# bogus2000/anytime-3D-reconstruction

Measured on AMD Instinct MI355X. Metric: 32^3 voxel reconstructions/sec at batch=256; IoU delta vs reference, higher is better.
Workload: dtype bf16

## Files before the change

anytime-3d-reconstruction_amd/csrc/skip_direct.hip:

```cpp
#include "common.h"

namespace {

typedef __attribute__((ext_vector_type(4))) unsigned sd_u4;

constexpr int SD_ATILE = 256 * 128;
constexpr int SD_WST = 32768;
constexpr int SD_A0 = 4096;
constexpr int SD_W0 = SD_A0 + 2 * SD_ATILE;
constexpr int SD_ZERO = SD_W0 + 2 * SD_WST;
constexpr int SD_LDS = SD_ZERO + 4096;
constexpr int SD_XCH = 0;
constexpr int SD_OST = 65536;
constexpr int SD_OPITCH = 144;
constexpr int SD_TPITCH = 272;
constexpr int SD_TWAVE = 16 * SD_TPITCH;

struct SdArgs {
    const void *x;
    const void *w;
    const float *scale;
    const float *shift;
    void *y;
    int batch, cin, cout, act;
    unsigned x_bytes, w_bytes;
    int groups;
};

__global__ void sd_pack_conv_kernel(const float *__restrict__ w, __bf16 *__restrict__ out, int cin, int cout) {
    const int NC = cin / 64;
    const long total = (long)64 * cin * cout;
    for (long i = (long)blockIdx.x * blockDim.x + threadIdx.x; i < total; i += (long)gridDim.x * blockDim.x) {
        const int k = (int)(i & 63);
        long r = i >> 6;
        const int n = (int)(r % cout); r /= cout;
        const int c = (int)(r % NC);
        const int t = (int)(r / NC);
        out[i] = static_cast<__bf16>(w[((size_t)t * cin + c * 64 + k) * cout + n]);
    }
}

__device__ __forceinline__ void sd_pack_conv_tiled_body(const float *__restrict__ w, __bf16 *__restrict__ out, int cin, int cout, int kb, int nb) {
    __shared__ float tile[64][65];
    const int tid = threadIdx.x;
    const int n0 = nb * 64;
    const int c4 = tid & 15, r = tid >> 4;
#pragma unroll
    for (int j = 0; j < 4; ++j) {
        const int kl = r + 16 * j;
// ... 43 lines not shown
        const int n = (int)(r % cout); r /= cout;
        const int c = (int)(r % NC); r /= NC;
        const int a = (int)(r & 7), p = (int)(r >> 3);
        const int td = 1 - ((p >> 2) & 1) + 2 * ((a >> 2) & 1);
        const int th = 1 - ((p >> 1) & 1) + 2 * ((a >> 1) & 1);
        const int tw = 1 - (p & 1) + 2 * (a & 1);
        const int t = (td * 4 + th) * 4 + tw;
        const float *src = w + ((size_t)t * cout + n) * cin + c * 64 + k;
        const f32x4 v0 = *reinterpret_cast<const f32x4 *>(src), v1 = *reinterpret_cast<const f32x4 *>(src + 4);
        bf16x8 o;
#pragma unroll
        for (int u = 0; u < 4; ++u) { o[u] = static_cast<__bf16>(v0[u]); o[4 + u] = static_cast<__bf16>(v1[u]); }
        *reinterpret_cast<bf16x8 *>(out + i8 * 8) = o;
    }
}

__global__ void sd_pack_convT_kernel(const float *__restrict__ w, __bf16 *__restrict__ out, int cin, int cout) {
    sd_pack_convT_body(w, out, cin, cout, blockIdx.x, gridDim.x);
}

__global__ void sd_pack_convT_multi_kernel(const SdPackJobs t) {
    int j = 0;
    while (j + 1 < t.njobs && (int)blockIdx.x >= t.first[j + 1]) ++j;
    sd_pack_convT_body(t.w[j], t.out[j], t.cin[j], t.cout[j], (int)blockIdx.x - t.first[j], t.first[j + 1] - t.first[j]);
}

#define SD_RD(DST, ADDR, OFF) asm volatile("ds_read_b128 %0, %1 offset:%2" : "=v"(DST) : "v"(ADDR), "n"(OFF) : "memory")
#define SD_WAIT8(N, F, G)                                                                                                   \
    asm volatile("s_waitcnt lgkmcnt(%8)"                                                                                    \
                 : "+v"(F[0]), "+v"(F[1]), "+v"(F[2]), "+v"(F[3]), "+v"(G[0]), "+v"(G[1]), "+v"(G[2]), "+v"(G[3])          \
                 : "n"(N)                                                                                                   \
                 : "memory")

template <int MODE>
__global__ __launch_bounds__(512, 1) void sd_kernel(const SdArgs a) {
    extern __shared__ __attribute__((aligned(16))) char smem[];
    const int tid = threadIdx.x, lane = tid & 63;
    const int wave = __builtin_amdgcn_readfirstlane(tid >> 6);
    const int mq = wave & 3, hv = wave >> 2;
    const int NC = a.cin >> 6;

    const int nwg = gridDim.x;
    const int wi = (nwg & 7) ? (int)blockIdx.x : (int)(blockIdx.x & 7) * (nwg >> 3) + (int)(blockIdx.x >> 3);
    const int sg = wi / a.groups, g = wi - sg * a.groups;
    const int b0 = sg * 4;
    const int ng = MODE == 0 ? g : (g >> 2);
    const int pd = (g >> 1) & 1, ph = g & 1;

    const u32x4 rsx = vv_make_rsrc(a.x, a.x_bytes), rsw = vv_make_rsrc(a.w, a.w_bytes);
    const unsigned lds0 = (unsigned)(unsigned long long)(lptr_t)smem;

    for (int i = tid; i < 256; i += 512) reinterpret_cast<uint4 *>(smem + SD_ZERO)[i] = make_uint4(0, 0, 0, 0);
    __syncthreads();

    unsigned a_lane[4], w_lane[4];
#pragma unroll
    for (int k = 0; k < 4; ++k) {
        const int it = wave * 4 + k;
        const int R = it * 8 + (lane >> 3);
        const int s = R >> 6, jd = (R >> 4) & 3, jh = (R >> 2) & 3, jw = R & 3;
        const int slot = (lane & 7) ^ (((s & 1) << 2) | (jw & 2));
        if (MODE == 0) a_lane[k] = (unsigned)(((((b0 + s) * 8 + 2 * jd) * 8 + 2 * jh) * 8 + 2 * jw) * (a.cin * 2) + slot * 16);
        else a_lane[k] = (unsigned)((((b0 + s) * 64) + (R & 63)) * (a.cin * 2) + slot * 16);
        const int blk = MODE == 0 ? (it & 7) : (it & 15);
        const int nrow = blk * 8 + (lane >> 3);
        w_lane[k] = (unsigned)(nrow * 128 + (((lane & 7) ^ ((nrow >> 1) & 7)) << 4));
    }
    auto issue_a = [&](int T, int tq, int tc) {
        unsigned soff;
        if (MODE == 0) {
            const int q = tq, c = tc;
            soff = (unsigned)(((1 - ((q >> 2) & 1)) * 64 + (1 - ((q >> 1) & 1)) * 8 + (1 - (q & 1))) * (a.cin * 2) + c * 128);
        } else {
            soff = (unsigned)(T * 128);
        }
        soff = __builtin_amdgcn_readfirstlane(soff);
        const unsigned dst = lds0 + SD_A0 + (T & 1) * SD_ATILE + wave * 4096;
#pragma unroll
        for (int k = 0; k < 4; ++k) vv_dma16(rsx, a_lane[k], soff, dst + k * 1024);
    };
    auto issue_w = [&](int u, int tq, int tc) {
        unsigned soff;
        if (MODE == 0) {
            const int ad = u & 1;
            const int q = tq, c = tc;
            const int j = wave >> 1;
            const int td = 2 * ad + ((q >> 2) & 1), th = 2 * (j >> 1) + ((q >> 1) & 1), tw = 2 * (j & 1) + (q & 1);
            const int t = (td * 4 + th) * 4 + tw;
            soff = (unsigned)(((t * NC + c) * a.cout + ng * 64) * 128);
        } else {
            const int c = u >> 3, ta = u & 7;
            const int p = pd * 4 + ph * 2 + hv;
            soff = (unsigned)((((p * 8 + ta) * NC + c) * a.cout + ng * 128) * 128);
        }
        soff = __builtin_amdgcn_readfirstlane(soff);
        const unsigned dst = lds0 + SD_W0 + (u & 1) * SD_WST + wave * 4096;
#pragma unroll
        for (int k = 0; k < 4; ++k) vv_dma16(rsw, w_lane[k], soff, dst + k * 1024);
    };

    const int r = lane & 15, kq = lane >> 4, ls = r >> 2, lw = r & 3;
    auto arow = [&](int jw, int ks) -> unsigned {
        const int f = ((ls & 1) << 2) | (jw & 2);
        return (unsigned)((ls * 64 + jw) * 128 + ((((ks << 2) | kq) ^ f) << 4));
    };
    unsigned wb[2];
#pragma unroll
    for (int ks = 0; ks < 2; ++ks) wb[ks] = lds0 + SD_W0 + (unsigned)(r * 128 + ((((ks << 2) | kq) ^ ((r >> 1) & 7)) << 4));
    const unsigned wbc = hv ? wb[1] : wb[0];
    const unsigned wbt0 = wb[0] + (unsigned)(hv * 16384), wbt1 = wb[1] + (unsigned)(hv * 16384);

    int td_[4], th_[4];
#pragma unroll
    for (int i = 0; i < 4; ++i) { td_[i] = i; th_[i] = (i + mq) & 3; }

    constexpr int NT = MODE == 0 ? 4 : 8;
    f32x4 acc[4][NT];
#pragma unroll
    for (int i = 0; i < 4; ++i)
#pragma unroll
        for (int j = 0; j < NT; ++j) acc[i][j] = f32x4{0.f, 0.f, 0.f, 0.f};

    auto mma4 = [&](const sd_u4 *xf, const sd_u4 *wf, int nt0, int vmask, auto i_c) {
        constexpr int i = decltype(i_c)::value;
        if (vmask & (1 << i)) {
#pragma unroll
            for (int j = 0; j < 4; ++j)
                acc[i][nt0 + j] = __builtin_amdgcn_mfma_f32_16x16x32_bf16(*reinterpret_cast<const bf16x8 *>(&wf[j]),
                                                                           *reinterpret_cast<const bf16x8 *>(&xf[i]), acc[i][nt0 + j], 0, 0, 0);
        }
    };
#define SD_MMA_RD(XF, WF, NT0, VM, R1, R2)                                                                                  \
    do {                                                                                                                    \
        mma4(XF, WF, NT0, VM, std::integral_constant<int, 0>{});                                                            \
        R1;                                                                                                                 \
        mma4(XF, WF, NT0, VM, std::integral_constant<int, 1>{});                                                            \
        R2;                                                                                                                 \
        mma4(XF, WF, NT0, VM, std::integral_constant<int, 2>{});                                                            \
        mma4(XF, WF, NT0, VM, std::integral_constant<int, 3>{});                                                            \
    } while (0)
    auto tile_mask = [&](const int *cell, int off) -> int {
        int m = 0;
#pragma unroll
        for (int i = 0; i < 4; ++i) m |= ((unsigned)(cell[i] + off) < 4u) ? (1 << i) : 0;
        return __builtin_amdgcn_readfirstlane(m);
    };

    const int ntiles = MODE == 0 ? 8 * NC : NC;
    const int nunits = ntiles * (MODE == 0 ? 2 : 8);

    const int q1_ = NC > 1 ? 0 : 1, c1_ = NC > 1 ? 1 : 0;
    issue_a(0, 0, 0);
    issue_w(0, 0, 0);
    if (ntiles > 1) issue_a(1, q1_, c1_); else issue_a(0, 0, 0);
    issue_w(1, 0, 0);
    vv_wait_vm<8>();
    __builtin_amdgcn_s_barrier();

    auto zrow = [&](int jw, int ks) -> unsigned { return lds0 + SD_ZERO + (arow(jw & 3, ks) & 255u); };

    sd_u4 xP[4], xQ[4], wP[4], wQ[4];
    if constexpr (MODE == 0) {
        const unsigned lm1 = arow((lw - 1) & 3, hv), l00 = arow(lw, hv), lp1 = arow((lw + 1) & 3, hv);
        const unsigned zm1 = zrow(lw - 1, hv), zp1 = zrow(lw + 1, hv);
        const bool okm1 = lw >= 1, okp1 = lw <= 2;
        unsigned xb0[4], xb1[4];
        int dm0, dm1, hm0, hm1;
        auto setup = [&](int T, int q) {
            const int qd = (q >> 2) & 1, qh = (q >> 1) & 1, qw = q & 1;
            const unsigned abuf = lds0 + SD_A0 + (T & 1) * SD_ATILE;
#pragma unroll
            for (int i = 0; i < 4; ++i) {
                const unsigned sc_ = abuf + (unsigned)((td_[i] - 1 + qd) * 2048 + (th_[i] - 1 + qh) * 512);
                xb0[i] = qw ? l00 + sc_ : (okm1 ? lm1 + sc_ : zm1);
                xb1[i] = qw ? (okp1 ? lp1 + sc_ : zp1) : l00 + sc_;
            }
            dm0 = tile_mask(td_, qd - 1); dm1 = tile_mask(td_, qd); hm0 = tile_mask(th_, qh - 1); hm1 = tile_mask(th_, qh);
        };
#define SD_CONV_RD(AD, J, XF, WF)                                                                                           \
    do {                                                                                                                    \
        constexpr int XO = (AD) * 2048 + ((J) >> 1) * 512, WO = (AD) * SD_WST + (J) * 8192;                                 \
        if ((J) & 1) { SD_RD(XF[0], xb1[0], XO); SD_RD(XF[1], xb1[1], XO); SD_RD(XF[2], xb1[2], XO); SD_RD(XF[3], xb1[3], XO); } \
        else { SD_RD(XF[0], xb0[0], XO); SD_RD(XF[1], xb0[1], XO); SD_RD(XF[2], xb0[2], XO); SD_RD(XF[3], xb0[3], XO); }     \
        SD_RD(WF[0], wbc, WO); SD_RD(WF[1], wbc, WO + 2048); SD_RD(WF[2], wbc, WO + 4096); SD_RD(WF[3], wbc, WO + 6144);    \
    } while (0)
#define SD_CONV_RDX(AD, J, XF)                                                                                              \
    do {                                                                                                                    \
        constexpr int XO = (AD) * 2048 + ((J) >> 1) * 512;                                                                  \
        if ((J) & 1) { SD_RD(XF[0], xb1[0], XO); SD_RD(XF[1], xb1[1], XO); SD_RD(XF[2], xb1[2], XO); SD_RD(XF[3], xb1[3], XO); } \
        else { SD_RD(XF[0], xb0[0], XO); SD_RD(XF[1], xb0[1], XO); SD_RD(XF[2], xb0[2], XO); SD_RD(XF[3], xb0[3], XO); }     \
    } while (0)
#define SD_CONV_RDW(AD, J, WF)                                                                                              \
    do {                                                                                                                    \
        constexpr int WO = (AD) * SD_WST + (J) * 8192;                                                                      \
        SD_RD(WF[0], wbc, WO); SD_RD(WF[1], wbc, WO + 2048); SD_RD(WF[2], wbc, WO + 4096); SD_RD(WF[3], wbc, WO + 6144);    \
    } while (0)
        setup(0, 0);
        SD_CONV_RD(0, 0, xP, wP);
        int qa = 0, ca = 0;
        int qb = q1_, cb = c1_;
        int qc = cb + 1 < NC ? qb : qb + 1, cc = cb + 1 < NC ? cb + 1 : 0;
#pragma unroll 1
        for (int T = 0; T < ntiles; ++T) {
            {
                const int u = 2 * T;
                SD_WAIT8(0, xP, wP);
                SD_MMA_RD(xP, wP, 0, dm0 & hm0, SD_CONV_RDX(0, 1, xQ), SD_CONV_RDW(0, 1, wQ));
                SD_WAIT8(0, xQ, wQ);
                SD_MMA_RD(xQ, wQ, 0, dm0 & hm0, SD_CONV_RDX(0, 2, xP), SD_CONV_RDW(0, 2, wP));
                SD_WAIT8(0, xP, wP);
                SD_MMA_RD(xP, wP, 0, dm0 & hm1, SD_CONV_RDX(0, 3, xQ), SD_CONV_RDW(0, 3, wQ));
                SD_WAIT8(0, xQ, wQ);
                vv_wait_vm<0>();
                __builtin_amdgcn_s_barrier();
                SD_MMA_RD(xQ, wQ, 0, dm0 & hm1, if (u + 2 < nunits) issue_w(u + 2, qb, cb); SD_CONV_RDX(1, 0, xP), SD_CONV_RDW(1, 0, wP));
            }
            {
                const int u = 2 * T + 1;
                SD_WAIT8(0, xP, wP);
                SD_MMA_RD(xP, wP, 0, dm1 & hm0, SD_CONV_RDX(1, 1, xQ), SD_CONV_RDW(1, 1, wQ));
                SD_WAIT8(0, xQ, wQ);
                SD_MMA_RD(xQ, wQ, 0, dm1 & hm0, SD_CONV_RDX(1, 2, xP), SD_CONV_RDW(1, 2, wP));
                SD_WAIT8(0, xP, wP);
                SD_MMA_RD(xP, wP, 0, dm1 & hm1, SD_CONV_RDX(1, 3, xQ), SD_CONV_RDW(1, 3, wQ));
                SD_WAIT8(0, xQ, wQ);
                vv_wait_vm<0>();
                __builtin_amdgcn_s_barrier();
                const int lastmask = dm1 & hm1;
                mma4(xQ, wQ, 0, lastmask, std::integral_constant<int, 0>{});
                if (u + 2 < nunits) issue_w(u + 2, qb, cb);
                if (T + 2 < ntiles) issue_a(T + 2, qc, cc);
                mma4(xQ, wQ, 0, lastmask, std::integral_constant<int, 1>{});
                if (T + 1 < ntiles) {
                    setup(T + 1, qb);
                    SD_CONV_RD(0, 0, xP, wP);
                }
                mma4(xQ, wQ, 0, lastmask, std::integral_constant<int, 2>{});
                mma4(xQ, wQ, 0, lastmask, std::integral_constant<int, 3>{});
            }
            qa = qb; ca = cb; qb = qc; cb = cc;
            qc = cb + 1 < NC ? qb : qb + 1; cc = cb + 1 < NC ? cb + 1 : 0;
            (void)qa; (void)ca;
        }
        asm volatile("s_waitcnt lgkmcnt(0)" ::: "memory");
        __builtin_amdgcn_sched_barrier(0);
#undef SD_CONV_RD
#undef SD_CONV_RDX
#undef SD_CONV_RDW
    } else {
        const int jw0 = lw + hv, jw1 = lw + hv - 1;
        const unsigned l0[2] = {arow(jw0 & 3, 0), arow(jw0 & 3, 1)}, l1[2] = {arow(jw1 & 3, 0), arow(jw1 & 3, 1)};
        const unsigned z0[2] = {zrow(jw0, 0), zrow(jw0, 1)}, z1[2] = {zrow(jw1, 0), zrow(jw1, 1)};
        const bool ok0 = (unsigned)jw0 < 4u, ok1 = (unsigned)jw1 < 4u;
        int dmA[2] = {tile_mask(td_, pd), tile_mask(td_, pd - 1)};
        const int hmA[2] = {tile_mask(th_, ph), tile_mask(th_, ph - 1)};
        unsigned xb[2][2][4];
        auto setup = [&](int T) {
            const unsigned abuf = lds0 + SD_A0 + (T & 1) * SD_ATILE;
#pragma unroll
            for (int i = 0; i < 4; ++i) {
                const unsigned sc_ = abuf + (unsigned)((td_[i] + pd - 1) * 2048 + (th_[i] + ph - 1) * 512);
#pragma unroll
                for (int ks = 0; ks < 2; ++ks) {
                    xb[0][ks][i] = ok0 ? l0[ks] + sc_ : z0[ks];
                    xb[1][ks][i] = ok1 ? l1[ks] + sc_ : z1[ks];
                }
            }
        };
#define SD_T_X(A, KS, XF)                                                                                                   \
    do {                                                                                                                    \
        constexpr int XO = (1 - (((A) >> 2) & 1)) * 2048 + (1 - (((A) >> 1) & 1)) * 512;                                    \
        SD_RD(XF[0], xb[(A) & 1][KS][0], XO); SD_RD(XF[1], xb[(A) & 1][KS][1], XO);                                         \
        SD_RD(XF[2], xb[(A) & 1][KS][2], XO); SD_RD(XF[3], xb[(A) & 1][KS][3], XO);                                         \
    } while (0)
#define SD_T_W(A, WB, HI, WF)                                                                                               \
    do {                                                                                                                    \
        constexpr int WO = ((A) & 1) * SD_WST + (HI) * 8192;                                                                \
        SD_RD(WF[0], WB, WO); SD_RD(WF[1], WB, WO + 2048); SD_RD(WF[2], WB, WO + 4096); SD_RD(WF[3], WB, WO + 6144);       \
    } while (0)
        setup(0);
        SD_T_X(0, 0, xP); SD_T_W(0, wbt0, 0, wP);
#pragma unroll 1
        for (int T = 0; T < ntiles; ++T) {
            auto unit = [&](auto a_c) {
                constexpr int A = decltype(a_c)::value;
                constexpr int AD = (A >> 2) & 1, AH = (A >> 1) & 1, AN = (A + 1) & 7;
                const int u = 8 * T + A;
                const int vm = dmA[AD] & hmA[AH];
                SD_WAIT8(0, xP, wP);
                SD_MMA_RD(xP, wP, 0, vm, SD_T_W(A, wbt0, 1, wQ), (void)0);
                SD_WAIT8(0, xP, wQ);
                SD_MMA_RD(xP, wQ, 4, vm, SD_T_X(A, 1, xQ), SD_T_W(A, wbt1, 0, wP));
                SD_WAIT8(0, xQ, wP);
                SD_MMA_RD(xQ, wP, 0, vm, SD_T_W(A, wbt1, 1, wQ), (void)0);
                SD_WAIT8(0, xQ, wQ);
                vv_wait_vm<0>();
                __builtin_amdgcn_s_barrier();
                mma4(xQ, wQ, 4, vm, std::integral_constant<int, 0>{});
                if (u + 2 < nunits) issue_w(u + 2, 0, 0);
                if (A == 7) {
                    if (T + 2 < ntiles) issue_a(T + 2, 0, 0);
                    mma4(xQ, wQ, 4, vm, std::integral_constant<int, 1>{});
                    if (T + 1 < ntiles) {
                        setup(T + 1);
                        SD_T_X(AN, 0, xP); SD_T_W(AN, wbt0, 0, wP);
                    }
                } else {
                    SD_T_X(AN, 0, xP);
                    mma4(xQ, wQ, 4, vm, std::integral_constant<int, 1>{});
                    SD_T_W(AN, wbt0, 0, wP);
                }
                mma4(xQ, wQ, 4, vm, std::integral_constant<int, 2>{});
                mma4(xQ, wQ, 4, vm, std::integral_constant<int, 3>{});
            };
            unit(std::integral_constant<int, 0>{});
            unit(std::integral_constant<int, 1>{});
            unit(std::integral_constant<int, 2>{});
            unit(std::integral_constant<int, 3>{});
            unit(std::integral_constant<int, 4>{});
            unit(std::integral_constant<int, 5>{});
            unit(std::integral_constant<int, 6>{});
            unit(std::integral_constant<int, 7>{});
        }
        asm volatile("s_waitcnt lgkmcnt(0)" ::: "memory");
        __builtin_amdgcn_sched_barrier(0);
#undef SD_T_X
#undef SD_T_W
    }
    __builtin_amdgcn_s_barrier();

    const int kq4 = kq * 4;
    if constexpr (MODE == 0) {
        f32x4 *xch = reinterpret_cast<f32x4 *>(smem + SD_XCH);
        {
            f32x4 *mine = xch + (size_t)wave * 8 * 64 + lane;
#pragma unroll
            for (int i = 0; i < 4; ++i)
#pragma unroll
                for (int j = 0; j < 2; ++j) mine[(i * 2 + j) * 64] = hv ? acc[i][j] : acc[i][2 + j];
        }
        __syncthreads();
        f32x4 fin[4][2];
        {
            const f32x4 *theirs = xch + (size_t)(wave ^ 4) * 8 * 64 + lane;
#pragma unroll
            for (int i = 0; i < 4; ++i)
#pragma unroll
                for (int j = 0; j < 2; ++j) fin[i][j] = (hv ? acc[i][2 + j] : acc[i][j]) + theirs[(i * 2 + j) * 64];
        }
        f32x4 sc[2], sh[2];
#pragma unroll
        for (int j = 0; j < 2; ++j) {
            const int n = ng * 64 + (2 * hv + j) * 16 + kq4;
            sc[j] = a.scale ? *reinterpret_cast<const f32x4 *>(a.scale + n) : f32x4{1.f, 1.f, 1.f, 1.f};
            sh[j] = a.shift ? *reinterpret_cast<const f32x4 *>(a.shift + n) : f32x4{0.f, 0.f, 0.f, 0.f};
        }
        auto fill = [&](auto act_c) {
            constexpr int ACT = decltype(act_c)::value;
#pragma unroll
            for (int i = 0; i < 4; ++i) {
                const int row = ls * 64 + td_[i] * 16 + th_[i] * 4 + lw;
#pragma unroll
                for (int j = 0; j < 2; ++j) {
                    bf16x4 o;
#pragma unroll
                    for (int e = 0; e < 4; ++e) {
                        float t = fin[i][j][e] * sc[j][e] + sh[j][e];
                        if (ACT == VV_ACT_ELU) { const float em = __expf(fminf(t, 0.f)) - 1.f; t = t > 0.f ? t : em; }
                        else if (ACT == VV_ACT_RELU) t = fmaxf(t, 0.f);
                        else if (ACT == VV_ACT_LRELU) t = t > 0.f ? t : 0.3f * t;
                        o[e] = static_cast<__bf16>(t);
                    }
                    *reinterpret_cast<bf16x4 *>(smem + SD_OST + row * SD_OPITCH + ((2 * hv + j) * 16 + kq4) * 2) = o;
                }
            }
        };
        VV_WITH_ACT(a.act, fill);
        __syncthreads();
#pragma unroll
        for (int k = 0; k < 4; ++k) {
            const int id = tid + 512 * k, row = id >> 3, pc = id & 7;
            const int b = b0 + (row >> 6);
            if (b < a.batch)
                *reinterpret_cast<uint4 *>(reinterpret_cast<char *>(a.y) + ((size_t)b * 64 + (row & 63)) * (a.cout * 2) + ng * 128 + pc * 16) =
                    *reinterpret_cast<const uint4 *>(smem + SD_OST + row * SD_OPITCH + pc * 16);
        }
    } else {
        char *mystage = smem + wave * SD_TWAVE;
        f32x4 sc[NT], sh[NT];
#pragma unroll
        for (int j = 0; j < NT; ++j) {
            const int n = ng * 128 + j * 16 + kq4;
            sc[j] = a.scale ? *reinterpret_cast<const f32x4 *>(a.scale + n) : f32x4{1.f, 1.f, 1.f, 1.f};
            sh[j] = a.shift ? *reinterpret_cast<const f32x4 *>(a.shift + n) : f32x4{0.f, 0.f, 0.f, 0.f};
        }
        auto fill = [&](auto act_c) {
            constexpr int ACT = decltype(act_c)::value;
#pragma unroll
            for (int i = 0; i < 4; ++i) {
#pragma unroll
                for (int j = 0; j < NT; ++j) {
                    bf16x4 o;
#pragma unroll
                    for (int e = 0; e < 4; ++e) {
                        float t = acc[i][j][e] * sc[j][e] + sh[j][e];
                        if (ACT == VV_ACT_ELU) { const float em = __expf(fminf(t, 0.f)) - 1.f; t = t > 0.f ? t : em; }
                        else if (ACT == VV_ACT_RELU) t = fmaxf(t, 0.f);
                        else if (ACT == VV_ACT_LRELU) t = t > 0.f ? t : 0.3f * t;
                        o[e] = static_cast<__bf16>(t);
                    }
                    *reinterpret_cast<bf16x4 *>(mystage + r * SD_TPITCH + (j * 16 + kq4) * 2) = o;
                }
                asm volatile("s_waitcnt lgkmcnt(0)" ::: "memory");
                __builtin_amdgcn_wave_barrier();
                const int od = 2 * td_[i] + pd, oh = 2 * th_[i] + ph;
#pragma unroll
                for (int k = 0; k < 4; ++k) {
                    const int id = lane + 64 * k, row = id >> 4, pc = id & 15;
                    const int b = b0 + (row >> 2), ow = 2 * (row & 3) + hv;
                    if (b < a.batch)
                        *reinterpret_cast<uint4 *>(reinterpret_cast<char *>(a.y) + ((((size_t)b * 8 + od) * 8 + oh) * 8 + ow) * (a.cout * 2) + ng * 256 + pc * 16) =
                            *reinterpret_cast<const uint4 *>(mystage + row * SD_TPITCH + pc * 16);
                }
                asm volatile("s_waitcnt lgkmcnt(0)" ::: "memory");
                __builtin_amdgcn_wave_barrier();
            }
        };
        VV_WITH_ACT(a.act, fill);
    }
}

template <int MODE>
int sd_launch(const void *x, const void *w, const float *scale, const float *shift, void *y, int batch, int cin, int cout, int act,
              hipStream_t st) {
    vv_allow_lds<&sd_kernel<MODE>>(SD_LDS);
    const size_t in_vox = MODE == 0 ? 512 : 64, out_vox = MODE == 0 ? 64 : 512;
    const size_t sample_in = in_vox * cin * 2, sample_out = out_vox * cout * 2;
    int per = (int)((0x7FFFFFFFull / sample_in) & ~3ull);
    if (per < 4) return VV_ERR_SHAPE;
    for (int s0 = 0; s0 < batch; s0 += per) {
        const int nb = batch - s0 < per ? batch - s0 : per;
        SdArgs a;
        a.x = reinterpret_cast<const char *>(x) + (size_t)s0 * sample_in;
        a.y = reinterpret_cast<char *>(y) + (size_t)s0 * sample_out;
        a.w = w; a.scale = scale; a.shift = shift;
        a.batch = nb; a.cin = cin; a.cout = cout; a.act = act;
        a.x_bytes = (unsigned)((size_t)nb * sample_in);
        a.w_bytes = (unsigned)((size_t)64 * cin * cout * 2);
        a.groups = MODE == 0 ? cout / 64 : 4 * (cout / 128);
        const int nsg = (nb + 3) / 4;
        VV_LAUNCH(sd_kernel<MODE>, dim3(nsg * a.groups), dim3(512), SD_LDS, st, a);
        const int rc = vv_launch_status();
        if (rc != VV_OK) return rc;
    }
    return VV_OK;
}

}

VV_EXPORT int vv_conv3d_k4s2_skip_supported(int side, int cin, int cout, int dtype) {
    return dtype == VV_BF16 && side == 8 && cin >= 64 && cin % 64 == 0 && cout >= 64 && cout % 64 == 0 && (size_t)64 * cin * cout * 2 < 0xFFFFFFF0ull;
}

VV_EXPORT int vv_convT3d_k4s2_skip_supported(int side, int cin, int cout, int dtype) {
    return dtype == VV_BF16 && side == 4 && cin >= 64 && cin % 64 == 0 && cout >= 128 && cout % 128 == 0 && (size_t)64 * cin * cout * 2 < 0xFFFFFFF0ull;
}

VV_EXPORT int vv_pack_conv_k4_skip(const float *w_keras, void *packed, int cin, int cout, void *stream) {
    if (!w_keras || !packed) return VV_ERR_NULL;
    if (cin <= 0 || cout <= 0 || cin % 64) return VV_ERR_SHAPE;
    if (cout % 64 == 0 && vv_aligned16(w_keras) && vv_aligned16(packed))
        VV_LAUNCH(sd_pack_conv_tiled_kernel, dim3(64 * (cin / 64), cout / 64), dim3(256), 0, reinterpret_cast<hipStream_t>(stream), w_keras,
                  reinterpret_cast<__bf16 *>(packed), cin, cout);
    else
        VV_LAUNCH(sd_pack_conv_kernel, dim3(vv_grid_1d((long)64 * cin * cout)), dim3(256), 0, reinterpret_cast<hipStream_t>(stream), w_keras,
                  reinterpret_cast<__bf16 *>(packed), cin, cout);
    return vv_launch_status();
}

VV_EXPORT int vv_pack_convT_k4s2_skip(const float *w_keras, void *packed, int cin, int cout, void *stream) {
    if (!w_keras || !packed) return VV_ERR_NULL;
    if (cin <= 0 || cout <= 0 || cin % 64) return VV_ERR_SHAPE;
    if (!vv_aligned16(w_keras) || !vv_aligned16(packed)) return VV_ERR_ALIGN;
    VV_LAUNCH(sd_pack_convT_kernel, dim3(vv_grid_1d((long)8 * cin * cout)), dim3(256), 0, reinterpret_cast<hipStream_t>(stream), w_keras,
              reinterpret_cast<__bf16 *>(packed), cin, cout);
    return vv_launch_status();
}

// ... 56 lines not shown
```

anytime-3d-reconstruction_amd/voxvae/isa_lint.py:

```python
import hashlib
import os
import re
import subprocess

PKG = os.path.dirname(os.path.dirname(os.path.abspath(__file__)))
ROOT = os.path.dirname(PKG)
CSRC = os.path.join(PKG, 'csrc')
ISA_DIR = os.path.join(PKG, 'lib', 'isa')
HIPCC = os.environ.get('HIPCC', '/opt/rocm/bin/hipcc')
FLAGS = ['--offload-arch=gfx950', '-O3', '-std=c++17', '-fPIC', '-fvisibility=hidden', '-w']

VM_OP = re.compile(r'^(buffer_|global_|flat_|scratch_|image_|tbuffer_)')
REG = re.compile(r'\b([va])(\d+)\b|\b([va])\[(\d+):(\d+)\]')


def compile_isa(src, force=False):
    os.makedirs(ISA_DIR, exist_ok=True)
    name = os.path.basename(src)[:-4]
    out = os.path.join(ISA_DIR, name + '.s')
    h = hashlib.sha256()
    deps = [src] + sorted(os.path.join(CSRC, f) for f in os.listdir(CSRC) if f.endswith('.h')) + [os.path.join(ROOT, 'include', 'voxvae.h')]
    for p in deps:
        with open(p, 'rb') as f:
            h.update(f.read())
# ... 164 lines not shown
    return res


def lint_file(src):
    fns = parse(compile_isa(src))
    out = {}
    for name, fn in fns.items():
        loads = asm_loads(fn)
        if not loads:
            continue
        r = {'loads': 0, 'dma': 0, 'violations': [], 'max_waits_vm': 0, 'max_waits_lgkm': 0, 'meta': fn['meta']}
        for idx, counter, dest in loads:
            w = walk(fn, idx, counter, dest)
            li = fn['ins'][idx]
            if dest is None:
                r['dma'] += 1
            else:
                r['loads'] += 1
            key = 'max_waits_vm' if counter == 'vm' else 'max_waits_lgkm'
            r[key] = max(r[key], w['waits'])
            for t in w['touched']:
                r['violations'].append('line %d `%s`: destination touched in flight at line %d `%s`' % (li.line, li.text, t.line, t.text))
        out[name] = r
    return out


PINNED_WAITS = {
    'conv_direct_kernel': (2, 2), 'conv_direct16_kernel': (2, 2), 'conv_direct16h_kernel': (2, 1), 'conv_direct_fp8_kernel': (2, 2),
    'convT_direct_kernel': (1, 2), 'convT_direct_fp8_kernel': (1, 2),
    'ctw_kernel': (4, 2), 'ctw16_kernel': (4, 2), 'ctw4_kernel': (4, 2),
    'final_bce_sweep_kernel': (3, 0), 'final_bce_sweepw_kernel': (3, 0), 'final_bce_sweep_fp8_kernel': (3, 0), 'final_bce_mfma_kernel': (0, 0),
    'final_mean_sweep_kernel': (2, 0),
    'igemm_kernel': (None, 0), 'pg_kernel': (None, 2), 'lt_e5_kernel': (1, 0),
    'sd_kernel': (2, 2), 'wgrad_bf16_kernel': (1, 1), 'wgrad_phase_kernel': (1, 2),
}
NO_SCRATCH = ('conv_direct_kernel', 'conv_direct16_kernel', 'conv_direct16h_kernel', 'conv_direct_fp8_kernel', 'convT_direct_fp8_kernel', 'ctw_kernel', 'ctw16_kernel',
              'final_bce_sweep_kernel', 'final_bce_sweepw_kernel', 'final_bce_sweep_fp8_kernel', 'final_mean_sweep_kernel', 'sd_kernel', 'pg_kernel', 'wgrad_phase_kernel', 'igemm_kernel')
RESIDENT_BUDGET = {'first_conv_chain_kernel': ('first_conv.hip', 128), 'final_bce_sweep_kernel': ('final_bce.hip', 168),
                   'final_bce_sweepw_kernel': ('final_bce.hip', 128)}


def family(mangled):
    m = re.match(r'^_ZN12_GLOBAL__N_1\d+([A-Za-z0-9_]+?_kernel)', mangled)
    return m.group(1) if m else mangled


def check_file(src):
    problems = []
    for kernel, r in lint_file(src).items():
        fam = family(kernel)
        for v in r['violations'][:4]:
            problems.append('%s: %s' % (kernel, v))
        if fam not in PINNED_WAITS:
            problems.append('new kernel with asm loads: add %s to PINNED_WAITS (vm %d, lgkm %d)' % (fam, r['max_waits_vm'], r['max_waits_lgkm']))
            continue
        vm, lg = PINNED_WAITS[fam]
        if vm is not None and r['max_waits_vm'] > vm:
            problems.append('%s: a look-ahead load now survives %d asm vmcnt waits (pinned %d)' % (kernel, r['max_waits_vm'], vm))
        if lg is not None and r['max_waits_lgkm'] > lg:
            problems.append('%s: an LDS read now survives %d asm lgkmcnt waits (pinned %d)' % (kernel, r['max_waits_lgkm'], lg))
        if fam in NO_SCRATCH and (r['meta'].get('private_segment_fixed_size', 0) or r['meta'].get('vgpr_spill_count', 0)):
            problems.append('%s: scratch / spills in a loop written for registers: %s' % (kernel, r['meta']))
    base = os.path.basename(src)
    for fam, (fsrc, budget) in RESIDENT_BUDGET.items():
        if fsrc != base:
            continue
        seen = False
# ... 34 lines not shown
```

anytime-3d-reconstruction_amd/voxvae/lib.py:

```python
import ctypes
import os

import torch

PKG = os.path.dirname(os.path.dirname(os.path.abspath(__file__)))
LIB_PATH = os.path.join(PKG, 'lib', 'libvoxvae.so')
HOOKS_LIB_PATH = os.path.join(PKG, 'lib', 'libvoxvae_hooks.so')
HOOK_VARS = ('VV_CD_SHAPE', 'VV_CDH_STAGGER', 'VV_CDH_ABL', 'VV_DIRECT_MT', 'VV_LT_KSLICE', 'VV_SPLIT_TARGET', 'VV_SPLIT_MINCHUNKS', 'VV_NO_KHALVES', 'VV_POSMAJOR_CONV_SIDE',
             'VV_POSMAJOR_CONVT_SIDE', 'VV_STAGES', 'VV_NO_FIRSTCONV', 'VV_WGRAD_F32', 'VV_PG_TARGET', 'VV_CTW_PS', 'VV_CTW_SHAPE',
             'VV_NO_WGRAD_PHASE', 'VV_BN_NB', 'VV_BN_SWEEP', 'VV_FINAL_BCE', 'VV_FIRSTCONV_GATHER', 'VV_FIRSTCONV_WGS', 'VV_FIRSTCONV_NOCHAIN', 'VV_CHUNK_SAMPLES', 'VV_C2_SPLITS')

VV_F32, VV_BF16, VV_FP8 = 0, 1, 2
VV_SCHED_LATENCY, VV_SCHED_THROUGHPUT = 0, 1
ACT = {None: 0, 'None': 0, 'linear': 0, 'elu': 1, 'relu': 2, 'lrelu': 3}
DTYPES = {'f32': VV_F32, 'fp32': VV_F32, 'float32': VV_F32, 'bf16': VV_BF16, 'bfloat16': VV_BF16, 'fp8': VV_FP8}

_vp, _i, _f, _sz, _l = ctypes.c_void_p, ctypes.c_int, ctypes.c_float, ctypes.c_size_t, ctypes.c_long
_u64 = ctypes.c_ulonglong

SIGNATURES = {
    'vv_abi_version': (_i, []),
    'vv_status_string': (ctypes.c_char_p, [_i]),
    'vv_last_hip_error': (ctypes.c_char_p, []),
    'vv_pack_conv_k4': (_i, [_vp, _vp, _i, _i, _i, _vp]),
    'vv_pack_convT_k4s2': (_i, [_vp, _vp, _i, _i, _i, _vp]),
    'vv_pack_conv_k4s1_meanpool': (_i, [_vp, _vp, _i, _i, _i, _i, _vp]),
    'vv_pack_conv_k4s1_full': (_i, [_vp, _vp, _i, _i, _i, _i, _vp]),
    'vv_max_over_positions': (_i, [_vp, _vp, _i, _i, _i, _vp]),
    'vv_sigmoid_f32': (_i, [_vp, _vp, _l, _vp]),
    'vv_pack_convT_k4s1_dense': (_i, [_vp, _vp, _i, _i, _i, _i, _vp]),
    'vv_pack_dense': (_i, [_vp, _vp, _i, _i, _i, _vp]),
    'vv_fold_bn': (_i, [_vp, _vp, _vp, _vp, _vp, _f, _vp, _vp, _i, _i, _vp]),
    'vv_conv3d_first_fwd': (_i, [_vp, _vp, _vp, _vp, _vp, _i, _i, _i, _i, _i, _vp]),
    'vv_conv3d_first_fwd_io': (_i, [_vp, _vp, _vp, _vp, _vp, _i, _i, _i, _i, _i, _i, _vp]),
    'vv_conv3d_k4s2_workspace_bytes': (_sz, [_i, _i, _i, _i, _i]),
    'vv_conv3d_k4s2_fwd': (_i, [_vp, _vp, _vp, _vp, _vp, _i, _i, _i, _i, _i, _i, _vp, _sz, _vp]),
    'vv_convT3d_k4s2_workspace_bytes': (_sz, [_i, _i, _i, _i, _i]),
    'vv_convT3d_k4s2_fwd': (_i, [_vp, _vp, _vp, _vp, _vp, _i, _i, _i, _i, _i, _i, _vp, _sz, _vp]),
    'vv_conv3d_k4s2_fwd_io': (_i, [_vp, _vp, _vp, _vp, _vp, _i, _i, _i, _i, _i, _i, _i, _vp, _sz, _vp]),
    'vv_convT3d_k4s2_fwd_io': (_i, [_vp, _vp, _vp, _vp, _vp, _i, _i, _i, _i, _i, _i, _i, _vp, _sz, _vp]),
    'vv_conv3d_k4s2_direct_supported': (_i, [_i, _i, _i, _i]),
    'vv_conv3d_k4s2_direct_fwd': (_i, [_vp, _vp, _vp, _vp, _vp, _i, _i, _i, _i, _i, _i, _vp]),
    'vv_conv3d_k4s2_direct_fwd_io': (_i, [_vp, _vp, _vp, _vp, _vp, _i, _i, _i, _i, _i, _i, _i, _vp]),
# ... 175 lines not shown
```

Before: 601,500.

## Use four-slot half-width weight ring and overlap zero-fill with prologue in skip conv

Refactors the skip-direct kernel into a FORM-templated body. For the conv mode (MODE 0) it defaults to a four-slot ring of half-size weight stages, which lets weight DMAs be issued earlier and waited on in finer steps, and it moves the LDS zero-row fill after the first DMA issues so the prologue overlaps. A batched convT epilogue that stages four cell tiles per wave before storing is added but only enabled through test hooks. The changes trade more complex waitcnt and barrier scheduling, plus higher vm-wait counts, for better overlap of global loads with MFMA work.

```diff
diff --git a/anytime-3d-reconstruction_amd/csrc/skip_direct.hip b/anytime-3d-reconstruction_amd/csrc/skip_direct.hip
--- a/anytime-3d-reconstruction_amd/csrc/skip_direct.hip
+++ b/anytime-3d-reconstruction_amd/csrc/skip_direct.hip
@@ -15,6 +15,11 @@
 constexpr int SD_OPITCH = 144;
 constexpr int SD_TPITCH = 272;
 constexpr int SD_TWAVE = 16 * SD_TPITCH;
+constexpr int SD_WHALF = SD_WST / 2;
+static_assert(8 * 4 * SD_TWAVE <= SD_LDS, "convT epilogue: every wave stages its four cell tiles at once");
+constexpr int SD_F_RING4 = 1;
+constexpr int SD_F_EDGES = 2;
+constexpr int sd_form(int mode) { return mode == 0 ? (SD_F_RING4 | SD_F_EDGES) : 0; }
 
 struct SdArgs {
     const void *x;
@@ -124,8 +129,9 @@
                  : "n"(N)                                                                                                   \
                  : "memory")
 
-template <int MODE>
-__global__ __launch_bounds__(512, 1) void sd_kernel(const SdArgs a) {
+template <int MODE, int FORM>
+__device__ __forceinline__ void sd_body(const SdArgs &a) {
+    constexpr bool RING4 = (FORM & SD_F_RING4) != 0, EDGES = (FORM & SD_F_EDGES) != 0;
     extern __shared__ __attribute__((aligned(16))) char smem[];
     const int tid = threadIdx.x, lane = tid & 63;
     const int wave = __builtin_amdgcn_readfirstlane(tid >> 6);
@@ -142,10 +148,17 @@
     const u32x4 rsx = vv_make_rsrc(a.x, a.x_bytes), rsw = vv_make_rsrc(a.w, a.w_bytes);
     const unsigned lds0 = (unsigned)(unsigned long long)(lptr_t)smem;
 
-    for (int i = tid; i < 256; i += 512) reinterpret_cast<uint4 *>(smem + SD_ZERO)[i] = make_uint4(0, 0, 0, 0);
-    __syncthreads();
-
-    unsigned a_lane[4], w_lane[4];
+    if constexpr (!EDGES) {
+        for (int i = tid; i < 256; i += 512) reinterpret_cast<uint4 *>(smem + SD_ZERO)[i] = make_uint4(0, 0, 0, 0);
+        __syncthreads();
+    }
+
+    unsigned a_lane[4], w_lane[4], w_lane4[2];
+#pragma unroll
+    for (int k = 0; k < 2; ++k) {
+        const int nrow = ((wave * 2 + k) & 7) * 8 + (lane >> 3);
+        w_lane4[k] = (unsigned)(nrow * 128 + (((lane & 7) ^ ((nrow >> 1) & 7)) << 4));
+    }
 #pragma unroll
     for (int k = 0; k < 4; ++k) {
         const int it = wave * 4 + k;
@@ -164,7 +177,7 @@
             const int q = tq, c = tc;
             soff = (unsigned)(((1 - ((q >> 2) & 1)) * 64 + (1 - ((q >> 1) & 1)) * 8 + (1 - (q & 1))) * (a.cin * 2) + c * 128);
         } else {
-            soff = (unsigned)(T * 128);
+            soff = (unsigned)(tc * 128);
         }
         soff = __builtin_amdgcn_readfirstlane(soff);
         const unsigned dst = lds0 + SD_A0 + (T & 1) * SD_ATILE + wave * 4096;
@@ -190,6 +203,23 @@
 #pragma unroll
         for (int k = 0; k < 4; ++k) vv_dma16(rsw, w_lane[k], soff, dst + k * 1024);
     };
+    auto issue_wh = [&](int slot, int half, int x0, int x1, int x2) {
+        unsigned soff;
+        if (MODE == 0) {
+            const int ad = x0, q = x1, c = x2;
+            const int td = 2 * ad + ((q >> 2) & 1), th = 2 * half + ((q >> 1) & 1), tw = 2 * (wave >> 2) + (q & 1);
+            const int t = (td * 4 + th) * 4 + tw;
+            soff = (unsigned)(((t * NC + c) * a.cout + ng * 64) * 128);
+        } else {
+            const int ta = x0, c = x1;
+            const int p = pd * 4 + ph * 2 + hv;
+            soff = (unsigned)((((p * 8 + ta) * NC + c) * a.cout + ng * 128 + half * 64) * 128);
+        }
+        soff = __builtin_amdgcn_readfirstlane(soff);
+        const unsigned dst = lds0 + SD_W0 + slot * SD_WHALF + wave * 2048;
+#pragma unroll
+        for (int k = 0; k < 2; ++k) vv_dma16(rsw, w_lane4[k], soff, dst + k * 1024);
+    };
 
     const int r = lane & 15, kq = lane >> 4, ls = r >> 2, lw = r & 3;
     auto arow = [&](int jw, int ks) -> unsigned {
@@ -200,7 +230,8 @@
 #pragma unroll
     for (int ks = 0; ks < 2; ++ks) wb[ks] = lds0 + SD_W0 + (unsigned)(r * 128 + ((((ks << 2) | kq) ^ ((r >> 1) & 7)) << 4));
     const unsigned wbc = hv ? wb[1] : wb[0];
-    const unsigned wbt0 = wb[0] + (unsigned)(hv * 16384), wbt1 = wb[1] + (unsigned)(hv * 16384);
+    constexpr int SD_WPAR = RING4 ? SD_WHALF / 2 : SD_WST / 2;
+    const unsigned wbt0 = wb[0] + (unsigned)(hv * SD_WPAR), wbt1 = wb[1] + (unsigned)(hv * SD_WPAR);
 
     int td_[4], th_[4];
 #pragma unroll
@@ -243,10 +274,24 @@
 
     const int q1_ = NC > 1 ? 0 : 1, c1_ = NC > 1 ? 1 : 0;
     issue_a(0, 0, 0);
-    issue_w(0, 0, 0);
-    if (ntiles > 1) issue_a(1, q1_, c1_); else issue_a(0, 0, 0);
-    issue_w(1, 0, 0);
-    vv_wait_vm<8>();
+    if constexpr (RING4) {
+        issue_wh(0, 0, 0, 0, 0); issue_wh(1, 1, 0, 0, 0);
+        issue_wh(2, 0, 1, 0, 0); issue_wh(3, 1, 1, 0, 0);
+        issue_a(1, q1_, c1_);
+    } else {
+        issue_w(0, 0, 0);
+        if (ntiles > 1) issue_a(1, q1_, c1_); else issue_a(0, 0, 0);
+        issue_w(1, 0, 0);
+    }
+    if constexpr (EDGES) {
+        for (int i = tid; i < 256; i += 512) reinterpret_cast<uint4 *>(smem + SD_ZERO)[i] = make_uint4(0, 0, 0, 0);
+        asm volatile("s_waitcnt lgkmcnt(0)" ::: "memory");
+    }
+    if constexpr (RING4) {
+        vv_wait_vm<10>();
+    } else {
+        vv_wait_vm<8>();
+    }
     __builtin_amdgcn_s_barrier();
 
     auto zrow = [&](int jw, int ks) -> unsigned { return lds0 + SD_ZERO + (arow(jw & 3, ks) & 255u); };
@@ -292,6 +337,58 @@
         int qa = 0, ca = 0;
         int qb = q1_, cb = c1_;
         int qc = cb + 1 < NC ? qb : qb + 1, cc = cb + 1 < NC ? cb + 1 : 0;
+        if constexpr (RING4) {
+            auto tile = [&](int T, auto last_c) {
+                constexpr bool LAST = decltype(last_c)::value;
+                SD_WAIT8(0, xP, wP);
+                SD_MMA_RD(xP, wP, 0, dm0 & hm0, SD_CONV_RDX(0, 1, xQ), SD_CONV_RDW(0, 1, wQ));
+                SD_WAIT8(0, xQ, wQ);
+                vv_wait_vm<8>();
+                __builtin_amdgcn_s_barrier();
+                SD_MMA_RD(xQ, wQ, 0, dm0 & hm0, if constexpr (!LAST) issue_wh(0, 0, 0, qb, cb); SD_CONV_RDX(0, 2, xP), SD_CONV_RDW(0, 2, wP));
+                SD_WAIT8(0, xP, wP);
+                SD_MMA_RD(xP, wP, 0, dm0 & hm1, SD_CONV_RDX(0, 3, xQ), SD_CONV_RDW(0, 3, wQ));
+                SD_WAIT8(0, xQ, wQ);
+                vv_wait_vm<LAST ? 6 : 8>();
+                __builtin_amdgcn_s_barrier();
+                SD_MMA_RD(xQ, wQ, 0, dm0 & hm1, if constexpr (!LAST) issue_wh(1, 1, 0, qb, cb); SD_CONV_RDX(1, 0, xP), SD_CONV_RDW(1, 0, wP));
+                SD_WAIT8(0, xP, wP);
+                SD_MMA_RD(xP, wP, 0, dm1 & hm0, SD_CONV_RDX(1, 1, xQ), SD_CONV_RDW(1, 1, wQ));
+                SD_WAIT8(0, xQ, wQ);
+                vv_wait_vm<LAST ? 4 : 8>();
+                __builtin_amdgcn_s_barrier();
+                SD_MMA_RD(xQ, wQ, 0, dm1 & hm0, if constexpr (!LAST) issue_wh(2, 0, 1, qb, cb); SD_CONV_RDX(1, 2, xP), SD_CONV_RDW(1, 2, wP));
+                SD_WAIT8(0, xP, wP);
+                SD_MMA_RD(xP, wP, 0, dm1 & hm1, SD_CONV_RDX(1, 3, xQ), SD_CONV_RDW(1, 3, wQ));
+                SD_WAIT8(0, xQ, wQ);
+                const int lastmask = dm1 & hm1;
+                if constexpr (!LAST) {
+                    vv_wait_vm<4>();
+                    __builtin_amdgcn_s_barrier();
+                    mma4(xQ, wQ, 0, lastmask, std::integral_constant<int, 0>{});
+                    issue_wh(3, 1, 1, qb, cb);
+                    const bool more = T + 2 < ntiles;
+                    issue_a(T + 2, more ? qc : qb, more ? cc : cb);
+                    mma4(xQ, wQ, 0, lastmask, std::integral_constant<int, 1>{});
+                    setup(T + 1, qb);
+                    SD_CONV_RD(0, 0, xP, wP);
+                } else {
+                    mma4(xQ, wQ, 0, lastmask, std::integral_constant<int, 0>{});
+                    mma4(xQ, wQ, 0, lastmask, std::integral_constant<int, 1>{});
+                }
+                mma4(xQ, wQ, 0, lastmask, std::integral_constant<int, 2>{});
+                mma4(xQ, wQ, 0, lastmask, std::integral_constant<int, 3>{});
+                if constexpr (LAST) vv_wait_vm<0>();
+            };
+            int T = 0;
+#pragma unroll 1
+            do {
+                tile(T, std::false_type{});
+                qb = qc; cb = cc;
+                qc = cb + 1 < NC ? qb : qb + 1; cc = cb + 1 < NC ? cb + 1 : 0;
+            } while (++T + 1 < ntiles);
+            tile(T, std::true_type{});
+        } else {
 #pragma unroll 1
         for (int T = 0; T < ntiles; ++T) {
             {
@@ -334,6 +431,7 @@
             qc = cb + 1 < NC ? qb : qb + 1; cc = cb + 1 < NC ? cb + 1 : 0;
             (void)qa; (void)ca;
         }
+        }
         asm volatile("s_waitcnt lgkmcnt(0)" ::: "memory");
         __builtin_amdgcn_sched_barrier(0);
 #undef SD_CONV_RD
@@ -370,7 +468,68 @@
         constexpr int WO = ((A) & 1) * SD_WST + (HI) * 8192;                                                                \
         SD_RD(WF[0], WB, WO); SD_RD(WF[1], WB, WO + 2048); SD_RD(WF[2], WB, WO + 4096); SD_RD(WF[3], WB, WO + 6144);       \
     } while (0)
+#define SD_T_W4(A, WB, HI, WF)                                                                                              \
+    do {                                                                                                                    \
+        constexpr int WO = (((A) & 1) * 2 + (HI)) * SD_WHALF;                                                               \
+        SD_RD(WF[0], WB, WO); SD_RD(WF[1], WB, WO + 2048); SD_RD(WF[2], WB, WO + 4096); SD_RD(WF[3], WB, WO + 6144);       \
+    } while (0)
         setup(0);
+        if constexpr (RING4) {
+            SD_T_X(0, 0, xP); SD_T_W4(0, wbt0, 0, wP);
+            auto unit4 = [&](int T, auto a_c, auto last_c) {
+                constexpr int A = decltype(a_c)::value;
+                constexpr bool LAST = decltype(last_c)::value;
+                static_assert(!LAST || A >= 6, "taps 0..5 are the same code in every tile");
+                constexpr int AD = (A >> 2) & 1, AH = (A >> 1) & 1, AN = (A + 1) & 7, A4 = (A + 2) & 7, SL = 2 * (A & 1);
+                constexpr bool ISSUE = !LAST;
+                constexpr int VM0 = LAST ? (A == 7 ? 0 : 4) : (A <= 1 ? 8 : 4), VM1 = LAST ? 2 : (A == 0 ? 8 : 4);
+                const int c4 = A >= 6 ? T + 1 : T;
+                const int vm = dmA[AD] & hmA[AH];
+                SD_WAIT8(0, xP, wP);
+                SD_MMA_RD(xP, wP, 0, vm, SD_T_X(A, 1, xQ), SD_T_W4(A, wbt1, 0, wQ));
+                SD_WAIT8(0, xQ, wQ);
+                vv_wait_vm<VM0>();
+                __builtin_amdgcn_s_barrier();
+                SD_MMA_RD(xQ, wQ, 0, vm, if constexpr (ISSUE) issue_wh(SL, 0, A4, c4, 0); SD_T_W4(A, wbt0, 1, wP), (void)0);
+                SD_WAIT8(0, xP, wP);
+                SD_MMA_RD(xP, wP, 4, vm, SD_T_W4(A, wbt1, 1, wQ), (void)0);
+                SD_WAIT8(0, xQ, wQ);
+                if constexpr (!(LAST && A == 7)) {
+                    vv_wait_vm<VM1>();
+                    __builtin_amdgcn_s_barrier();
+                }
+                mma4(xQ, wQ, 4, vm, std::integral_constant<int, 0>{});
+                if constexpr (ISSUE) issue_wh(SL + 1, 1, A4, c4, 0);
+                if constexpr (A == 7) {
+                    if constexpr (!LAST) issue_a(T + 2, 0, T + 2 < ntiles ? T + 2 : T + 1);
+                    mma4(xQ, wQ, 4, vm, std::integral_constant<int, 1>{});
+                    if constexpr (!LAST) {
+                        setup(T + 1);
+                        SD_T_X(AN, 0, xP); SD_T_W4(AN, wbt0, 0, wP);
+                    }
+                } else {
+                    SD_T_X(AN, 0, xP);
+                    mma4(xQ, wQ, 4, vm, std::integral_constant<int, 1>{});
+                    SD_T_W4(AN, wbt0, 0, wP);
+                }
+                mma4(xQ, wQ, 4, vm, std::integral_constant<int, 2>{});
+                mma4(xQ, wQ, 4, vm, std::integral_constant<int, 3>{});
+            };
+            auto tile4 = [&](int T, auto last_c) {
+                unit4(T, std::integral_constant<int, 0>{}, std::false_type{});
+                unit4(T, std::integral_constant<int, 1>{}, std::false_type{});
+                unit4(T, std::integral_constant<int, 2>{}, std::false_type{});
+                unit4(T, std::integral_constant<int, 3>{}, std::false_type{});
+                unit4(T, std::integral_constant<int, 4>{}, std::false_type{});
+                unit4(T, std::integral_constant<int, 5>{}, std::false_type{});
+                unit4(T, std::integral_constant<int, 6>{}, last_c);
+                unit4(T, std::integral_constant<int, 7>{}, last_c);
+            };
+            int T = 0;
+#pragma unroll 1
+            for (; T + 1 < ntiles; ++T) tile4(T, std::false_type{});
+            tile4(T, std::true_type{});
+        } else {
         SD_T_X(0, 0, xP); SD_T_W(0, wbt0, 0, wP);
 #pragma unroll 1
         for (int T = 0; T < ntiles; ++T) {
@@ -391,7 +550,7 @@
                 mma4(xQ, wQ, 4, vm, std::integral_constant<int, 0>{});
                 if (u + 2 < nunits) issue_w(u + 2, 0, 0);
                 if (A == 7) {
-                    if (T + 2 < ntiles) issue_a(T + 2, 0, 0);
+                    if (T + 2 < ntiles) issue_a(T + 2, 0, T + 2);
                     mma4(xQ, wQ, 4, vm, std::integral_constant<int, 1>{});
                     if (T + 1 < ntiles) {
                         setup(T + 1);
@@ -414,10 +573,12 @@
             unit(std::integral_constant<int, 6>{});
             unit(std::integral_constant<int, 7>{});
         }
+        }
         asm volatile("s_waitcnt lgkmcnt(0)" ::: "memory");
         __builtin_amdgcn_sched_barrier(0);
 #undef SD_T_X
 #undef SD_T_W
+#undef SD_T_W4
     }
     __builtin_amdgcn_s_barrier();
 
@@ -478,7 +639,7 @@
                     *reinterpret_cast<const uint4 *>(smem + SD_OST + row * SD_OPITCH + pc * 16);
         }
     } else {
-        char *mystage = smem + wave * SD_TWAVE;
+        char *mystage = smem + wave * (EDGES ? 4 * SD_TWAVE : SD_TWAVE);
         f32x4 sc[NT], sh[NT];
 #pragma unroll
         for (int j = 0; j < NT; ++j) {
@@ -486,6 +647,17 @@
             sc[j] = a.scale ? *reinterpret_cast<const f32x4 *>(a.scale + n) : f32x4{1.f, 1.f, 1.f, 1.f};
             sh[j] = a.shift ? *reinterpret_cast<const f32x4 *>(a.shift + n) : f32x4{0.f, 0.f, 0.f, 0.f};
         }
+        auto store_tile = [&](int i, const char *stage) {
+            const int od = 2 * td_[i] + pd, oh = 2 * th_[i] + ph;
+#pragma unroll
+            for (int k = 0; k < 4; ++k) {
+                const int id = lane + 64 * k, row = id >> 4, pc = id & 15;
+                const int b = b0 + (row >> 2), ow = 2 * (row & 3) + hv;
+                if (b < a.batch)
+                    *reinterpret_cast<uint4 *>(reinterpret_cast<char *>(a.y) + ((((size_t)b * 8 + od) * 8 + oh) * 8 + ow) * (a.cout * 2) + ng * 256 + pc * 16) =
+                        *reinterpret_cast<const uint4 *>(stage + row * SD_TPITCH + pc * 16);
+            }
+        };
         auto fill = [&](auto act_c) {
             constexpr int ACT = decltype(act_c)::value;
 #pragma unroll
@@ -501,21 +673,21 @@
                         else if (ACT == VV_ACT_LRELU) t = t > 0.f ? t : 0.3f * t;
                         o[e] = static_cast<__bf16>(t);
                     }
-                    *reinterpret_cast<bf16x4 *>(mystage + r * SD_TPITCH + (j * 16 + kq4) * 2) = o;
+                    *reinterpret_cast<bf16x4 *>(mystage + (EDGES ? i * SD_TWAVE : 0) + r * SD_TPITCH + (j * 16 + kq4) * 2) = o;
                 }
+                if constexpr (!EDGES) {
+                    asm volatile("s_waitcnt lgkmcnt(0)" ::: "memory");
+                    __builtin_amdgcn_wave_barrier();
+                    store_tile(i, mystage);
+                    asm volatile("s_waitcnt lgkmcnt(0)" ::: "memory");
+                    __builtin_amdgcn_wave_barrier();
+                }
+            }
+            if constexpr (EDGES) {
                 asm volatile("s_waitcnt lgkmcnt(0)" ::: "memory");
                 __builtin_amdgcn_wave_barrier();
-                const int od = 2 * td_[i] + pd, oh = 2 * th_[i] + ph;
-#pragma unroll
-                for (int k = 0; k < 4; ++k) {
-                    const int id = lane + 64 * k, row = id >> 4, pc = id & 15;
-                    const int b = b0 + (row >> 2), ow = 2 * (row & 3) + hv;
-                    if (b < a.batch)
-                        *reinterpret_cast<uint4 *>(reinterpret_cast<char *>(a.y) + ((((size_t)b * 8 + od) * 8 + oh) * 8 + ow) * (a.cout * 2) + ng * 256 + pc * 16) =
-                            *reinterpret_cast<const uint4 *>(mystage + row * SD_TPITCH + pc * 16);
-                }
-                asm volatile("s_waitcnt lgkmcnt(0)" ::: "memory");
-                __builtin_amdgcn_wave_barrier();
+#pragma unroll
+                for (int i = 0; i < 4; ++i) store_tile(i, mystage + i * SD_TWAVE);
             }
         };
         VV_WITH_ACT(a.act, fill);
@@ -523,9 +695,20 @@
 }
 
 template <int MODE>
-int sd_launch(const void *x, const void *w, const float *scale, const float *shift, void *y, int batch, int cin, int cout, int act,
-              hipStream_t st) {
-    vv_allow_lds<&sd_kernel<MODE>>(SD_LDS);
+__global__ __launch_bounds__(512, 1) void sd_kernel(const SdArgs a) {
+    sd_body<MODE, sd_form(MODE)>(a);
+}
+#ifdef VV_TEST_HOOKS
+template <int MODE, int FORM>
+__global__ __launch_bounds__(512, 1) void sd_kernel_form(const SdArgs a) {
+    sd_body<MODE, FORM>(a);
+}
+#endif
+
+template <int MODE, auto Kernel>
+int sd_launch_form(const void *x, const void *w, const float *scale, const float *shift, void *y, int batch, int cin, int cout, int act,
+                   hipStream_t st) {
+    vv_allow_lds<Kernel>(SD_LDS);
     const size_t in_vox = MODE == 0 ? 512 : 64, out_vox = MODE == 0 ? 64 : 512;
     const size_t sample_in = in_vox * cin * 2, sample_out = out_vox * cout * 2;
     int per = (int)((0x7FFFFFFFull / sample_in) & ~3ull);
@@ -541,11 +724,28 @@
         a.w_bytes = (unsigned)((size_t)64 * cin * cout * 2);
         a.groups = MODE == 0 ? cout / 64 : 4 * (cout / 128);
         const int nsg = (nb + 3) / 4;
-        VV_LAUNCH(sd_kernel<MODE>, dim3(nsg * a.groups), dim3(512), SD_LDS, st, a);
+        VV_LAUNCH(Kernel, dim3(nsg * a.groups), dim3(512), SD_LDS, st, a);
         const int rc = vv_launch_status();
         if (rc != VV_OK) return rc;
     }
     return VV_OK;
+}
+
+template <int MODE>
+int sd_launch(const void *x, const void *w, const float *scale, const float *shift, void *y, int batch, int cin, int cout, int act,
+              hipStream_t st) {
+#ifdef VV_TEST_HOOKS
+    constexpr int DEF = sd_form(MODE);
+    const int form = (vv_hook_int(vv_hook("VV_SD_RING"), (DEF & SD_F_RING4) ? 4 : 2) == 4 ? SD_F_RING4 : 0) |
+                     (vv_hook_int(vv_hook("VV_SD_EDGES"), (DEF & SD_F_EDGES) ? 1 : 0) != 0 ? SD_F_EDGES : 0);
+    if (form != DEF) {
+        if (form == 0) return sd_launch_form<MODE, &sd_kernel_form<MODE, 0>>(x, w, scale, shift, y, batch, cin, cout, act, st);
+        if (form == 1) return sd_launch_form<MODE, &sd_kernel_form<MODE, 1>>(x, w, scale, shift, y, batch, cin, cout, act, st);
+        if (form == 2) return sd_launch_form<MODE, &sd_kernel_form<MODE, 2>>(x, w, scale, shift, y, batch, cin, cout, act, st);
+        return sd_launch_form<MODE, &sd_kernel_form<MODE, 3>>(x, w, scale, shift, y, batch, cin, cout, act, st);
+    }
+#endif
+    return sd_launch_form<MODE, &sd_kernel<MODE>>(x, w, scale, shift, y, batch, cin, cout, act, st);
 }
 
 }
diff --git a/anytime-3d-reconstruction_amd/voxvae/isa_lint.py b/anytime-3d-reconstruction_amd/voxvae/isa_lint.py
--- a/anytime-3d-reconstruction_amd/voxvae/isa_lint.py
+++ b/anytime-3d-reconstruction_amd/voxvae/isa_lint.py
@@ -220,7 +220,7 @@
     'final_bce_sweep_kernel': (3, 0), 'final_bce_sweepw_kernel': (3, 0), 'final_bce_sweep_fp8_kernel': (3, 0), 'final_bce_mfma_kernel': (0, 0),
     'final_mean_sweep_kernel': (2, 0),
     'igemm_kernel': (None, 0), 'pg_kernel': (None, 2), 'lt_e5_kernel': (1, 0),
-    'sd_kernel': (2, 2), 'wgrad_bf16_kernel': (1, 1), 'wgrad_phase_kernel': (1, 2),
+    'sd_kernel': (5, 2), 'wgrad_bf16_kernel': (1, 1), 'wgrad_phase_kernel': (1, 2),
 }
 NO_SCRATCH = ('conv_direct_kernel', 'conv_direct16_kernel', 'conv_direct16h_kernel', 'conv_direct_fp8_kernel', 'convT_direct_fp8_kernel', 'ctw_kernel', 'ctw16_kernel',
               'final_bce_sweep_kernel', 'final_bce_sweepw_kernel', 'final_bce_sweep_fp8_kernel', 'final_mean_sweep_kernel', 'sd_kernel', 'pg_kernel', 'wgrad_phase_kernel', 'igemm_kernel')
diff --git a/anytime-3d-reconstruction_amd/voxvae/lib.py b/anytime-3d-reconstruction_amd/voxvae/lib.py
--- a/anytime-3d-reconstruction_amd/voxvae/lib.py
+++ b/anytime-3d-reconstruction_amd/voxvae/lib.py
@@ -8,7 +8,8 @@
 HOOKS_LIB_PATH = os.path.join(PKG, 'lib', 'libvoxvae_hooks.so')
 HOOK_VARS = ('VV_CD_SHAPE', 'VV_CDH_STAGGER', 'VV_CDH_ABL', 'VV_DIRECT_MT', 'VV_LT_KSLICE', 'VV_SPLIT_TARGET', 'VV_SPLIT_MINCHUNKS', 'VV_NO_KHALVES', 'VV_POSMAJOR_CONV_SIDE',
              'VV_POSMAJOR_CONVT_SIDE', 'VV_STAGES', 'VV_NO_FIRSTCONV', 'VV_WGRAD_F32', 'VV_PG_TARGET', 'VV_CTW_PS', 'VV_CTW_SHAPE',
-             'VV_NO_WGRAD_PHASE', 'VV_BN_NB', 'VV_BN_SWEEP', 'VV_FINAL_BCE', 'VV_FIRSTCONV_GATHER', 'VV_FIRSTCONV_WGS', 'VV_FIRSTCONV_NOCHAIN', 'VV_CHUNK_SAMPLES', 'VV_C2_SPLITS')
+             'VV_NO_WGRAD_PHASE', 'VV_BN_NB', 'VV_BN_SWEEP', 'VV_FINAL_BCE', 'VV_FIRSTCONV_GATHER', 'VV_FIRSTCONV_WGS', 'VV_FIRSTCONV_NOCHAIN', 'VV_CHUNK_SAMPLES', 'VV_C2_SPLITS',
+             'VV_SD_RING', 'VV_SD_EDGES')
 
 VV_F32, VV_BF16, VV_FP8 = 0, 1, 2
 VV_SCHED_LATENCY, VV_SCHED_THROUGHPUT = 0, 1
```

Result: no change. 599,300 (-0.4%).
